# sxyu/volrend

Measured on AMD Instinct MI355X. Metric: Mrays/s at 800x800, NeRF-synthetic-like SH16 (synthetic C1), higher is better.
Workload: dtype f32; 1 GPU; C1: synthetic lego-like PlenOctree, depth 9, SH16, 2025715 nodes, 2.24 GB in HBM, 800x800, fx=fy=1111.111, 200-pose orbit, default RenderOptions; fp_mode=strict, launches=38, pcie_inclusive=False, launch_streams=1, parallelism=single GPU

## Files before the change

### include/volrend_hip.h

```cpp
#ifndef VOLREND_HIP_H_
#define VOLREND_HIP_H_

#include <stddef.h>
#include <stdint.h>

#ifdef __cplusplus
extern "C" {
#endif

#define VR_ABI_VERSION 3

enum {
    VR_OK = 0,
    VR_ERR_INVALID_ARGUMENT = 1,
    VR_ERR_HIP = 2,
    VR_ERR_NO_DEVICE = 3,
    VR_ERR_BAD_TREE = 4,
    VR_ERR_UNSUPPORTED = 5,
    VR_ERR_OUT_OF_MEMORY = 6
};

enum { VR_FORMAT_RGBA = 0, VR_FORMAT_SH = 1, VR_FORMAT_SG = 2, VR_FORMAT_ASG = 3 };

enum { VR_FP_STRICT = 0, VR_FP_FMA = 1 };
// ... 258 lines not shown
    int          bits;
    uint32_t*    order;
    uint32_t*    keys;
    float*       origins_out;
    float*       dirs_out;
    const float* payload;
    float*       payload_out;
    int          payload_dim;
} VrRayOrder;
int64_t vr_order_rays_workspace(int64_t n);
int vr_order_rays(vr_tree_t tree, int64_t n, const VrRays* rays, const VrRenderOptions* opt, int fp_mode,
                  const VrRayOrder* out, void* workspace, size_t workspace_bytes, void* stream);
int vr_reserve_rays(vr_tree_t tree, int64_t n, int n_slots);
int vr_reserve(vr_tree_t tree, int width, int height, int n_frames);
int vr_reserve_tiles(vr_tree_t tree, int width, int height, int n_frames, int tile_w, int tile_h,
                     int world, int n_slots);
int vr_tree_status(vr_tree_t tree, uint32_t* status, int reset);
int vr_tree_status_on(vr_tree_t tree, uint32_t* status, int reset, void* stream);
int vr_set_tuning(const char* key, int value);
int vr_tree_set_tuning(vr_tree_t tree, const char* key, int value);
int vr_sched_stats(vr_tree_t tree, uint64_t out[8], int reset);
int vr_tree_cull_stats(vr_tree_t tree, uint64_t out[2], int reset);
int vr_tree_head_stats(vr_tree_t tree, uint64_t out[3], int reset);
int vr_touch_enable(vr_tree_t tree, int enable);
int vr_touch_count(vr_tree_t tree, uint64_t out[4], int reset);
int vr_touch_read(vr_tree_t tree, int which, uint32_t* host_words, uint64_t n_words,
                  uint64_t* bitmap_words, uint64_t* granule_bytes);
int vr_assemble_tiles(void* frame_rgba, int64_t pitch, const void* gathered, int width,
                      int height, int tile_w, int tile_h, int world, void* stream);
int vr_assemble_tiles_batch(void* frames_rgba, int64_t frame_stride, int64_t pitch,
                            const void* gathered, int64_t rank_stride, int64_t in_frame_stride,
                            int n_frames, int width, int height, int tile_w, int tile_h, int world,
                            void* stream);
int vr_probe_coeffs(vr_tree_t tree, const VrRenderOptions* opt, float* out_dev, void* stream);

enum { VR_SPACE_WORLD = 0, VR_SPACE_TREE = 1 };

typedef struct VrQueryOut {
    float* sigma;
    int32_t* depth;
    float* local;
    float* coeffs;
    float* rgb;
} VrQueryOut;

int vr_query_points(vr_tree_t tree, int64_t n, const float* xyz_dev, const float* dirs_dev, int space,
// ... 13 lines not shown
```

### volrend_amd/_abi.py

```python
from __future__ import annotations

import ctypes as C
import os

HERE = os.path.dirname(os.path.abspath(__file__))
LIB_PATH = os.environ.get("VOLREND_HIP_LIB") or os.path.join(HERE, "libvolrend_hip.so")

VR_OK = 0
FORMAT_RGBA, FORMAT_SH, FORMAT_SG, FORMAT_ASG = 0, 1, 2, 3
FORMATS = {"RGBA": FORMAT_RGBA, "SH": FORMAT_SH, "SG": FORMAT_SG, "ASG": FORMAT_ASG}
FP_STRICT, FP_FMA = 0, 1
QUERY_LOOKUP, QUERY_DESCENT = 0, 1
LAYOUT_FRAME, LAYOUT_COMPACT = 0, 1
SPACE_WORLD, SPACE_TREE = 0, 1
SPACES = {"world": SPACE_WORLD, "tree": SPACE_TREE}
DEPTH_TREE, DEPTH_WORLD = 0, 1
DEPTH_UNITS = {"tree": DEPTH_TREE, "world": DEPTH_WORLD}
DATA_F16, DATA_F32 = 0, 1
STEP_SGD, STEP_ADAM = 0, 1
STEP_KINDS = {"sgd": STEP_SGD, "adam": STEP_ADAM}
MAX_BASIS = 25
ORDER_MAX_BITS, ORDER_MAX_PAYLOAD = 5, 8
REFINE_COPY, REFINE_ZERO = 0, 1
REFINE_FILLS = {"copy": REFINE_COPY, "zero": REFINE_ZERO}
# ... 173 lines not shown
    "vr_slot_points": (C.c_int, [C.POINTER(VrSlotPoints), C.c_void_p]),
    "vr_render_rays": (C.c_int, [C.c_void_p, C.c_int64, C.POINTER(VrRays), C.POINTER(VrRenderOptions), C.c_int,
                                 C.POINTER(VrRayOut), C.c_void_p]),
    "vr_accumulate_weights_rays": (C.c_int, [C.c_void_p, C.c_int64, C.POINTER(VrRays), C.POINTER(VrRenderOptions),
                                             C.c_int, C.POINTER(VrLeafWeights), C.c_void_p]),
    "vr_render_backward_rays": (C.c_int, [C.c_void_p, C.c_int64, C.POINTER(VrRays), C.POINTER(VrRenderOptions),
                                          C.c_int, C.c_void_p, C.c_void_p, C.c_void_p]),
    "vr_fit_rays": (C.c_int, [C.c_void_p, C.c_int64, C.POINTER(VrRays), C.POINTER(VrRenderOptions), C.c_int,
                              C.POINTER(VrFit), C.c_void_p]),
    "vr_order_rays_workspace": (C.c_int64, [C.c_int64]),
    "vr_order_rays": (C.c_int, [C.c_void_p, C.c_int64, C.POINTER(VrRays), C.POINTER(VrRenderOptions), C.c_int,
                                C.POINTER(VrRayOrder), C.c_void_p, C.c_size_t, C.c_void_p]),
    "vr_reserve_rays": (C.c_int, [C.c_void_p, C.c_int64, C.c_int]),
    "vr_reserve": (C.c_int, [C.c_void_p, C.c_int, C.c_int, C.c_int]),
    "vr_reserve_tiles": (C.c_int, [C.c_void_p, C.c_int, C.c_int, C.c_int, C.c_int, C.c_int, C.c_int,
                                   C.c_int]),
    "vr_tree_status": (C.c_int, [C.c_void_p, C.POINTER(C.c_uint32), C.c_int]),
    "vr_tree_status_on": (C.c_int, [C.c_void_p, C.POINTER(C.c_uint32), C.c_int, C.c_void_p]),
    "vr_set_tuning": (C.c_int, [C.c_char_p, C.c_int]),
    "vr_tree_set_tuning": (C.c_int, [C.c_void_p, C.c_char_p, C.c_int]),
    "vr_sched_stats": (C.c_int, [C.c_void_p, C.POINTER(C.c_uint64 * 8), C.c_int]),
    "vr_tree_cull_stats": (C.c_int, [C.c_void_p, C.POINTER(C.c_uint64 * 2), C.c_int]),
    "vr_tree_head_stats": (C.c_int, [C.c_void_p, C.POINTER(C.c_uint64 * 3), C.c_int]),
    "vr_touch_enable": (C.c_int, [C.c_void_p, C.c_int]),
    "vr_touch_count": (C.c_int, [C.c_void_p, C.POINTER(C.c_uint64 * 4), C.c_int]),
    "vr_touch_read": (C.c_int, [C.c_void_p, C.c_int, C.c_void_p, C.c_uint64, C.POINTER(C.c_uint64),
                                C.POINTER(C.c_uint64)]),
    "vr_assemble_tiles": (C.c_int, [C.c_void_p, C.c_int64, C.c_void_p, C.c_int, C.c_int, C.c_int,
                                    C.c_int, C.c_int, C.c_void_p]),
    "vr_assemble_tiles_batch": (C.c_int, [C.c_void_p, C.c_int64, C.c_int64, C.c_void_p, C.c_int64,
                                          C.c_int64, C.c_int, C.c_int, C.c_int, C.c_int, C.c_int,
                                          C.c_int, C.c_void_p]),
    "vr_probe_coeffs": (C.c_int, [C.c_void_p, C.POINTER(VrRenderOptions), C.c_void_p, C.c_void_p]),
    "vr_query_points": (C.c_int, [C.c_void_p, C.c_int64, C.c_void_p, C.c_void_p, C.c_int,
                                  C.POINTER(VrQueryOut), C.c_void_p]),
    "vr_query_grid": (C.c_int, [C.c_void_p, C.POINTER(C.c_float * 3), C.POINTER(C.c_float * 3),
                                C.POINTER(C.c_int32 * 3), C.POINTER(C.c_float * 3), C.c_int,
                                C.POINTER(VrQueryOut), C.c_void_p]),
    "vr_read_back": (C.c_int, [C.c_void_p, C.c_void_p, C.c_int64, C.c_int, C.c_int, C.c_void_p]),
    "vr_stream_sync": (C.c_int, [C.c_void_p]),
}

_lib = None


class VolrendError(RuntimeError):
# ... 27 lines not shown
```

### volrend_amd/_tree.py

```python
from __future__ import annotations

import ctypes as C
import os

import numpy as np

from . import _abi, _ops
from ._args import F16, I32, Buf, _stream_ptr, check


class _CurrentDevice:

    def info(self) -> dict:
        import torch
        return {"device": int(torch.cuda.current_device())}


def parse_data_format(s: str):
    idx = next((i for i, ch in enumerate(s) if not ch.isalpha()), -1)
    if idx < 0:
        return "RGBA", -1
    head = s[:idx]
    try:
        dim = int("".join(ch for ch in s[idx:] if ch.isdigit() or ch == "-") or "0")
# ... 211 lines not shown
        return self._loaded

    def clear_cpu_memory(self) -> None:
        self.data_ = None
        self.quant_ = None

    def sched_stats(self, reset: bool = True) -> dict:
        out = (C.c_uint64 * 8)()
        _abi.check(_abi.lib().vr_sched_stats(self._handle, C.byref(out), 1 if reset else 0))
        names = ("march_rounds", "march_lanes", "shade_rounds", "shade_lanes", "distinct_leaves",
                 "retire_rounds", "retired", "iterations")
        return dict(zip(names, [int(v) for v in out]))

    def cull_stats(self, reset: bool = True) -> dict:
        out = (C.c_uint64 * 2)()
        _abi.check(_abi.lib().vr_tree_cull_stats(self.handle, C.byref(out), 1 if reset else 0))
        return {"blocks": int(out[0]), "culled": int(out[1])}

    def head_stats(self, reset: bool = False) -> dict:
        out = (C.c_uint64 * 3)()
        _abi.check(_abi.lib().vr_tree_head_stats(self.handle, C.byref(out), 1 if reset else 0))
        return {"entered": int(out[0]), "retired": int(out[1]), "samples": int(out[2])}

    def touch_enable(self, enable: bool = True) -> None:
        _abi.check(_abi.lib().vr_touch_enable(self.handle, 1 if enable else 0))

    def touch_count(self, reset: bool = True) -> dict:
        out = (C.c_uint64 * 4)()
        _abi.check(_abi.lib().vr_touch_count(self.handle, C.byref(out), 1 if reset else 0))
        return dict(zip(("leaves", "nodes", "top", "bricks"), [int(v) for v in out]))

    def touch_read(self, which: int):
        words, gran = C.c_uint64(0), C.c_uint64(0)
        _abi.check(_abi.lib().vr_touch_read(self.handle, int(which), None, 0, C.byref(words), C.byref(gran)))
        out = np.zeros(int(words.value), dtype=np.uint32)
        if out.size:
            _abi.check(_abi.lib().vr_touch_read(self.handle, int(which), out.ctypes.data, out.size, None, None))
        return out, int(gran.value)

    def reserve(self, width: int, height: int, n_frames: int, shard: "TileShard | None" = None,
                n_slots: int = 2) -> None:
        if shard is None and n_slots == 2:
            _abi.check(_abi.lib().vr_reserve(self.handle, int(width), int(height), int(n_frames)))
        else:
            tw, th, world = (shard.tile_w, shard.tile_h, shard.world) if shard else (0, 0, 1)
            _abi.check(_abi.lib().vr_reserve_tiles(self.handle, int(width), int(height),
# ... 88 lines not shown
```

### volrend_amd/build.py

```python
from __future__ import annotations

import os
import shutil
import subprocess
import sys
import tempfile

HERE = os.path.dirname(os.path.abspath(__file__))
ROOT = os.path.dirname(HERE)
CSRC = os.path.join(HERE, "csrc")
LIB = os.path.join(HERE, "libvolrend_hip.so")
SOURCES = ["vr_render.hip", "vr_weights.hip", "vr_grad.hip", "vr_fit.hip", "vr_update.hip", "vr_tree_kernels.hip", "vr_query.hip", "vr_order.hip", "vr_refine.hip", "vr_collapse.hip", "vr_geometry.hip", "vr_api.cpp", "vr_upload.cpp", "vr_tree_walk.cpp",
           "vr_h2d.cpp", "vr_launch.cpp", "vr_launch_plan.cpp", "vr_slots.cpp", "vr_values.cpp", "vr_query.cpp", "vr_order.cpp", "vr_refine.cpp", "vr_collapse.cpp", "vr_geometry.cpp"]
HEADERS = ["vr_internal.h", "vr_device_math.h", "vr_host.h", "vr_dev_layout.h", "vr_dev_shade.h", "vr_dev_query.h",
           "vr_dev_rays.h", "vr_dev_march.h", "vr_dev_backward.h", "vr_query.h", "vr_order.h", "vr_refine.h", "vr_collapse.h", "vr_geometry.h", "vr_tree_walk.h", "vr_launch_plan.h", "vr_h2d.h", os.path.join(ROOT, "include", "volrend_hip.h"),
           os.path.join(ROOT, "include", "volrend", "internal", "hip_owners.hpp")]
EXPERIMENTS = os.path.join(ROOT, "tools", "experiments")
HOOK_FLAGS = ("-DVR_ABLATE", "-DVR_TIMELINE", "-DVR_ROLE_DEBUG", "-DVR_MIN_WAVES_PER_EU", "-DVR_SH16_ROWS",
              "-DVR_SHADE_SCHED_BARRIER", "-DVR_SH16_WAVES", "-DVR_SH25_WAVES", "-DVR_SH9_WAVES", "-DVR_PACKED_EXP",
              "-DVR_STEAL_MIN", "-DVR_EXP_SH25_STRIDE", "-DVR_TOUCH_LEAF_SHIFT")
HIPCC = os.environ.get("HIPCC", "/opt/rocm/bin/hipcc")
FLAGS = [
    "--offload-arch=gfx950", "-O3", "-std=c++17", "-fPIC", "-shared",
    "-ffp-contract=off",
    "-fhip-fp32-correctly-rounded-divide-sqrt",
    "-fno-gpu-flush-denormals-to-zero",
    "-fno-fast-math",
    "-x", "hip",
]


def needs_build() -> bool:
    if not os.path.exists(LIB):
        return True
    t = os.path.getmtime(LIB)
    deps = [os.path.join(CSRC, s) for s in SOURCES] + [
        h if os.path.isabs(h) else os.path.join(CSRC, h) for h in HEADERS]
    return any(os.path.getmtime(d) > t for d in deps)
# ... 48 lines not shown
```

### volrend_amd/csrc/vr_api.cpp

```cpp
#include <hip/hip_runtime.h>

#include <climits>
#include <cstdarg>
#include <cstdio>
#include <cstdlib>
#include <cstring>
#include <mutex>

#include "vr_host.h"
#include "vr_tree_walk.h"

namespace {

thread_local char g_err[512] = "";

enum KnobRange { kClamp, kClamp64, kFlag, kAutoFlag };
struct Knob { const char *key, *env; int Tuning::*field; KnobRange range; int lo, hi; bool fixed_at_upload; };
const Knob kKnobs[] = {
    {"march_max", "VR_MARCH_MAX", &Tuning::march_max, kClamp, 1, INT_MAX, false},
    {"refill_min", "VR_REFILL_MIN", &Tuning::refill_min, kClamp, 1, 64, false},
    {"drain_flush", "VR_DRAIN_FLUSH", &Tuning::drain_flush, kClamp, 0, 64, false},
    {"waves_per_cu", "VR_WAVES_PER_CU", &Tuning::waves_per_cu, kClamp, 0, 64, false},
    {"frame_group", "VR_FRAME_GROUP", &Tuning::frame_group, kClamp, 0, INT_MAX, false},
    {"super_block", "VR_SUPER_BLOCK", &Tuning::super_block, kClamp, 0, 64, false},
// ... 189 lines not shown
    HIP_TRY(hipMemcpy(lines, t->cull_stats.get(), sizeof(lines), hipMemcpyDeviceToHost));
    if (reset) HIP_TRY(hipMemset(t->cull_stats.get(), 0, sizeof(lines)));
    out[0] = out[1] = 0;
    for (int i = 0; i < vr::kCullStatLines; ++i) {
        out[0] += lines[i * vr::kCullStatStride];
        out[1] += lines[i * vr::kCullStatStride + 1];
    }
    return VR_OK;
}

int vr_tree_head_stats(vr_tree_t t, uint64_t out[3], int reset) {
    if (!t || !out) return fail(VR_ERR_INVALID_ARGUMENT, "NULL argument");
    DeviceGuard guard(t->device);
    uint64_t lines[vr::kCullStatLines * vr::kCullStatStride];
    HIP_TRY(hipMemcpy(lines, t->head_stats.get(), sizeof(lines), hipMemcpyDeviceToHost));
    if (reset) HIP_TRY(hipMemset(t->head_stats.get(), 0, sizeof(lines)));
    for (int k = 0; k < vr::kHeadStatWords; ++k) {
        out[k] = 0;
        for (int i = 0; i < vr::kCullStatLines; ++i) out[k] += lines[i * vr::kCullStatStride + k];
    }
    return VR_OK;
}

int vr_tree_status(vr_tree_t t, uint32_t* status, int reset) {
    if (!t || !status) return fail(VR_ERR_INVALID_ARGUMENT, "NULL argument");
    DeviceGuard guard(t->device);
    HIP_TRY(hipMemcpy(status, t->status.get(), sizeof(uint32_t), hipMemcpyDeviceToHost));
    if (reset) HIP_TRY(hipMemset(t->status.get(), 0, sizeof(uint32_t)));
    return VR_OK;
}

int vr_tree_status_on(vr_tree_t t, uint32_t* status, int reset, void* stream) {
    if (!t || !status) return fail(VR_ERR_INVALID_ARGUMENT, "NULL argument");
    DeviceGuard guard(t->device);
    hipStream_t hs = static_cast<hipStream_t>(stream);
    thread_local uint32_t* pinned = nullptr;
    if (!pinned) HIP_TRY(hipHostMalloc((void**)&pinned, sizeof(uint32_t), hipHostMallocPortable));
    HIP_TRY(hipMemcpyAsync(pinned, t->status.get(), sizeof(uint32_t), hipMemcpyDeviceToHost, hs));
    if (reset) HIP_TRY(hipMemsetAsync(t->status.get(), 0, sizeof(uint32_t), hs));
    HIP_TRY(hipStreamSynchronize(hs));
    *status = *pinned;
    return VR_OK;
}

int vr_touch_enable(vr_tree_t t, int enable) {
    if (!t) return fail(VR_ERR_INVALID_ARGUMENT, "tree is NULL");
// ... 103 lines not shown
```

### volrend_amd/csrc/vr_dev_march.h

```cpp
#pragma once
#include <type_traits>
#include "vr_device_math.h"
#include "vr_internal.h"
#include "vr_dev_layout.h"
#include "vr_dev_query.h"
#include "vr_dev_rays.h"

namespace vr {

namespace {

enum { kQueryN2 = 0, kQueryN2Blocked = 1, kQueryGeneric = 2 };
inline int query_kind(const KParams& p) {
    return !uses_lookup(p) ? kQueryGeneric : (p.brick_blocked ? kQueryN2Blocked : kQueryN2);
}
template <typename F>
void dispatch_query(int query, F&& f) {
    if (query == kQueryGeneric) f(std::integral_constant<int, kQueryGeneric>());
    else if (query == kQueryN2Blocked) f(std::integral_constant<int, kQueryN2Blocked>());
    else f(std::integral_constant<int, kQueryN2>());
}

struct WeightRecord {
    static constexpr int kWords = kWeightRayWords;
    static constexpr bool kShade = false;
};
struct GradRecord {
    static constexpr int kWords = kGradRayWords;
    static constexpr bool kShade = true;
};

template <int GW, typename Record>
__device__ __forceinline__ void store_march_record(const KParams& p, bool valid, int lane, int wave, const Ray& nr,
                                                   const float* vdir, uint32_t pixel) {
    const unsigned long long m_valid = __builtin_amdgcn_ballot_w64(valid);
    const uint32_t my_base = reserve_ray_slots<GW>(p, m_valid, lane, wave);
    if (!valid) return;
    uint32_t* rb = ray_slot(p.ray_buf_rw, Record::kWords, my_base + lane_rank(m_valid));
    store_march_words(rb, nr);
    if constexpr (Record::kShade) {
#pragma unroll
        for (int i = 0; i < 3; ++i) ray_word(rb, kGradRayVdir + i) = f2u(vdir[i]);
        ray_word(rb, kGradRayPixel) = pixel;
    }
}

template <int FMA, int GW, typename Record>
__global__ __launch_bounds__(kWave* GW) void march_raygen_kernel(const KParams p) {
    const int lane = threadIdx.x & (kWave - 1);
    const int wave = threadIdx.x >> 6;
    const uint32_t id = (uint32_t)(((int64_t)blockIdx.x * GW + wave) * kWave + lane);
    bool valid = false;
    Ray nr;
    nr.alive = false;
    float vdir[3] = {0.f, 0.f, 0.f};
    uint32_t pixel = 0;
    if (id < p.total_rays) {
        const PixelRef r = locate(p, id);
        if (r.in_image) {
            setup_ray<FMA>(p, r, nr, vdir);
            valid = nr.alive;
            pixel = ((uint32_t)r.frame * (uint32_t)p.height + (uint32_t)r.y) * (uint32_t)p.width + (uint32_t)r.x;
        }
    }
    store_march_record<GW, Record>(p, valid, lane, wave, nr, vdir, pixel);
}

template <int FMA, int GW, typename Record>
__global__ __launch_bounds__(kWave* GW) void march_raygen_rays_kernel(const KParams p, const RayList rl) {
    const int lane = threadIdx.x & (kWave - 1);
    const int wave = threadIdx.x >> 6;
    uint32_t id;
    Ray nr;
    float vdir[3] = {0.f, 0.f, 0.f};
    const bool valid = list_ray<FMA, GW>(p, rl, lane, wave, id, nr, vdir) && nr.alive;
    store_march_record<GW, Record>(p, valid, lane, wave, nr, vdir, id);
}

template <typename Launch>
void launch_raygen_waves(const KParams& p, int gen_waves, Launch&& launch) {
    const int gw = gen_waves >= 16 ? 16 : 4;
    const dim3 grid((unsigned)((p.n_wave_blocks * p.n_frames + gw - 1) / gw)), block(kWave * gw);
    if (gw == 16) launch(std::integral_constant<int, 16>(), grid, block);
    else launch(std::integral_constant<int, 4>(), grid, block);
}
template <int FMA, typename Record>
void launch_march_raygen(const KParams& p, int gen_waves, hipStream_t s, const RayList* rays) {
    launch_raygen_waves(p, gen_waves, [&](auto gw, dim3 grid, dim3 block) {
        constexpr int GW = decltype(gw)::value;
        if (rays) hipLaunchKernelGGL((march_raygen_rays_kernel<FMA, GW, Record>), grid, block, 0, s, p, *rays);
        else hipLaunchKernelGGL((march_raygen_kernel<FMA, GW, Record>), grid, block, 0, s, p);
    });
}

struct MarchFeed {
    bool exhausted;
    uint32_t chunk_next, chunk_end;
    uint32_t progress_round;
};
// ... 132 lines not shown
```

### volrend_amd/csrc/vr_dev_rays.h

```cpp
#pragma once
#include "vr_device_math.h"
#include "vr_dev_layout.h"
#include "vr_dev_shade.h"

namespace vr {

namespace {

struct RayCounters {
    uint32_t samples = 0, child_reads = 0, hits = 0, early = 0, entered = 0;
};

typedef __attribute__((address_space(1))) uint32_t vr_gword_t;
typedef float vr_f4_t __attribute__((ext_vector_type(4)));
typedef __attribute__((address_space(1))) vr_f4_t vr_gfloat4_t;

__device__ __forceinline__ bool wave_any(bool v) { return __builtin_amdgcn_ballot_w64(v) != 0ull; }
__device__ __forceinline__ uint32_t lane_id_now() {
    uint32_t l;
    asm volatile("v_mbcnt_lo_u32_b32 %0, -1, 0\n\tv_mbcnt_hi_u32_b32 %0, -1, %0" : "=v"(l));
    return l;
}
__device__ __forceinline__ uint32_t lane_rank(unsigned long long mask) {
    return __builtin_amdgcn_mbcnt_hi((uint32_t)(mask >> 32), __builtin_amdgcn_mbcnt_lo((uint32_t)mask, 0u));
}

// ... 265 lines not shown
            const uint32_t x = (mine + a) & (nq - 1u);
            uint32_t* const q = p.queue_head + x * kQueueStride;
            uint32_t* const head = q + kQueueHead;
            const uint32_t len = q[kQueueCount];
            const uint32_t seen = __hip_atomic_load(head, __ATOMIC_RELAXED, __HIP_MEMORY_SCOPE_AGENT);
            if (seen >= len) continue;
            if (a != 0u && gridDim.x >= nq &&
                len - seen < ((len >> 3) < kStealMin ? (len >> 3) : kStealMin))
                continue;
            uint32_t size = (len - seen) / (2u * waves_per_q);
            size = size < 64u ? 64u : (size > (uint32_t)p.chunk_max ? (uint32_t)p.chunk_max : size);
            size &= ~63u;
            const uint32_t base = atomicAdd(head, size);
            if (base < len) {
                const uint32_t qlo = queue_first_block(n16, x, sh) << 6;
                lo = qlo + base;
                hi = qlo + (base + size < len ? base + size : len);
                break;
            }
        }
    }
}

template <int GW>
__device__ __forceinline__ uint32_t reserve_ray_slots(const KParams& p, unsigned long long m_valid, int lane,
                                                      int wave) {
    __shared__ uint32_t wave_count[GW];
    __shared__ uint32_t wave_base[GW];
    const uint32_t nq = (uint32_t)p.n_queues;
    uint32_t sh, n16;
    queue_split(p, sh, n16);
    const uint32_t g16 = (uint32_t)(((int64_t)blockIdx.x * GW) >> 4);
    uint32_t qx = (uint32_t)(((uint64_t)g16 << sh) / n16);
    while (qx + 1u < nq && (queue_first_block(n16, qx + 1u, sh) >> 4) <= g16) ++qx;
    while (qx > 0u && (queue_first_block(n16, qx, sh) >> 4) > g16) --qx;
    uint32_t* const q_count = p.queue_head + qx * kQueueStride + kQueueCount;
    const uint32_t q_base = queue_first_block(n16, qx, sh) << 6;
    if constexpr (GW == 1) {
        const uint32_t n = (uint32_t)__builtin_popcountll(m_valid);
        uint32_t b = 0;
        if (lane == 0 && n) b = atomicAdd(q_count, n);
        return q_base + (uint32_t)__builtin_amdgcn_readfirstlane((int)b);
    } else {
        if (lane == 0) wave_count[wave] = (uint32_t)__builtin_popcountll(m_valid);
        __syncthreads();
        if (threadIdx.x == 0) {
            uint32_t sum = 0;
#pragma unroll
            for (int w = 0; w < GW; ++w) {
                wave_base[w] = sum;
                sum += wave_count[w];
            }
            const uint32_t base = q_base + (sum ? atomicAdd(q_count, sum) : 0u);
#pragma unroll
            for (int w = 0; w < GW; ++w) wave_base[w] += base;
        }
        __syncthreads();
        return wave_base[wave];
    }
}

__device__ __forceinline__ void store_march_words(uint32_t* rb, const Ray& nr) {
#pragma unroll
    for (int i = 0; i < 3; ++i) {
        ray_word(rb, kRayCen + i) = f2u(nr.cen[i]);
        ray_word(rb, kRayDir + i) = f2u(nr.dir[i]);
        ray_word(rb, kRayInvDir + i) = f2u(nr.invdir[i]);
    }
    ray_word(rb, kRayT) = f2u(nr.t);
    ray_word(rb, kRayTmax) = f2u(nr.tmax);
    ray_word(rb, kRayDeltaScale) = f2u(nr.delta_scale);
}

template <int FMA, int GW>
__device__ __forceinline__ bool list_ray(const KParams& p, const RayList& rl, int lane, int wave, uint32_t& id,
                                         Ray& ray, float* vdir) {
    typedef __attribute__((address_space(1))) const float vr_gcfloat_t;
    __shared__ float tr[GW][2][3 * kWave];
    const int64_t first = ((int64_t)blockIdx.x * GW + wave) * kWave;
    const int64_t left = rl.n - first;
    const int count = left <= 0 ? 0 : (left < kWave ? (int)left : kWave);
    vr_gcfloat_t* const so = (vr_gcfloat_t*)rl.origins + first * 3;
    vr_gcfloat_t* const sd = (vr_gcfloat_t*)rl.dirs + first * 3;
#pragma unroll
    for (int c = 0; c < 3; ++c) {
        const int f = c * kWave + lane;
        if (f < count * 3) {
            tr[wave][0][f] = so[f];
            tr[wave][1][f] = sd[f];
        }
    }
    __syncthreads();
    id = (uint32_t)first + (uint32_t)lane;
    reset_ray(ray);
    if (lane >= count) return false;
    if (p.N <= 0) return true;
    float cen[3], dir[3];
#pragma unroll
    for (int c = 0; c < 3; ++c) {
        cen[c] = tr[wave][0][lane * 3 + c];
        dir[c] = tr[wave][1][lane * 3 + c];
    }
// ... 9 lines not shown
```

### volrend_amd/csrc/vr_fit.hip

```cpp
#include "vr_dev_backward.h"

namespace vr {

namespace {

__device__ __forceinline__ void loss_head(const FitParams& fp, uint32_t i, const float* out, float* g) {
    vr_gcfloat_t* const tg = (vr_gcfloat_t*)fp.target + (size_t)i * 3u;
    const float na = 1.f - out[3];
    float r[3];
#pragma unroll
    for (int ch = 0; ch < 3; ++ch) {
        const float pred = out[ch] + fp.bg * na;
        r[ch] = pred - tg[ch];
    }
    if (fp.sq_err) ((vr_gfloat_t*)fp.sq_err)[i] = (r[0] * r[0] + r[1] * r[1]) + r[2] * r[2];
    if (fp.accum) ((vr_gfloat4_t*)fp.accum)[i] = (vr_f4_t){out[0], out[1], out[2], out[3]};
#pragma unroll
    for (int ch = 0; ch < 3; ++ch) g[ch] = fp.grad_scale * r[ch];
    g[3] = -(fp.bg * ((g[0] + g[1]) + g[2]));
}

template <int FMA, int GW>
__global__ __launch_bounds__(kWave* GW) void fit_raygen_kernel(const KParams p, const RayList rl, const FitParams fp) {
    const int lane = threadIdx.x & (kWave - 1);
    const int wave = threadIdx.x >> 6;
    uint32_t id;
    Ray nr;
    float vdir[3] = {0.f, 0.f, 0.f};
    const bool has = list_ray<FMA, GW>(p, rl, lane, wave, id, nr, vdir);
    const bool valid = has && nr.alive;
    if (has && !valid) {
        const float out[4] = {0.f, 0.f, 0.f, 0.f};
        float g[4];
        loss_head(fp, id, out, g);
    }
    store_march_record<GW, GradRecord>(p, valid, lane, wave, nr, vdir, id);
}

struct FitArgs : FitParams {
    static constexpr bool kFit = true, kMark = true;
    explicit FitArgs(const FitParams& f) : FitParams(f) {}
};

template <int FMA>
hipError_t launch_fp(const KParams& p, const FitParams& fp, int n_cus, int waves_override, int gen_waves, hipStream_t s,
                     const RayList& rays) {
    launch_raygen_waves(p, gen_waves, [&](auto gw, dim3 grid, dim3 block) {
        hipLaunchKernelGGL((fit_raygen_kernel<FMA, decltype(gw)::value>), grid, block, 0, s, p, rays, fp);
    });
    return launch_backward_march<FMA>(p, FitArgs(fp), n_cus, waves_override, s);
}

}

hipError_t launch_fit(const KParams& p, const FitParams& fp, int fp_mode, int n_cus, int waves_override, int gen_waves,
                      hipStream_t stream, const RayList* rays) {
    if (p.n_wave_blocks <= 0 || p.n_frames <= 0 || !rays) return hipSuccess;
    return fp_mode == VR_FP_FMA ? launch_fp<1>(p, fp, n_cus, waves_override, gen_waves, stream, *rays)
                                : launch_fp<0>(p, fp, n_cus, waves_override, gen_waves, stream, *rays);
// ... 4 lines not shown
```

### volrend_amd/csrc/vr_host.h

```cpp
#pragma once
#include <hip/hip_runtime.h>

#include <mutex>
#include <vector>

#include "vr_internal.h"
#include "vr_launch_plan.h"

#pragma GCC visibility push(hidden)

#include "volrend/internal/hip_owners.hpp"
using volrend::internal::DeviceBuffer;
using volrend::internal::DeviceEvent;
using volrend::internal::DeviceGuard;

int fail(int code, const char* fmt, ...);
inline int hip_code(hipError_t e) { return e == hipErrorOutOfMemory ? VR_ERR_OUT_OF_MEMORY : VR_ERR_HIP; }

#define HIP_TRY(expr)                                                                                 \
    do {                                                                                              \
        hipError_t e_ = (expr);                                                                       \
        if (e_ != hipSuccess)                                                                         \
            return fail(hip_code(e_), "%s failed: %s (%s:%d)", #expr, hipGetErrorString(e_), __FILE__, \
                        __LINE__);                                                                    \
// ... 23 lines not shown
    uint64_t device_bytes = 0;
};

struct VrTreeOpaque : TreeShape {
    int device = 0;
    DeviceBuffer arrays[4];
    DeviceBuffer extra, status, sched_stats;
    DeviceBuffer occ;
    DeviceBuffer cull_stats;
    DeviceBuffer head_stats;
    DeviceBuffer touch[4];
    DeviceBuffer touch_out;
    DeviceBuffer probe_buf;
    DeviceBuffer slot_frames;
    DeviceBuffer slot_heads;
    DeviceBuffer slot_aovs;
    std::vector<int32_t> file_node;
    DeviceBuffer file_node_dev;
    std::vector<int32_t> brick_root;
    DeviceBuffer brick_root_dev;
    DeviceBuffer node_of_file_dev;
    LaunchSlot slots[kLaunchSlots];
    unsigned launch_seq = 0;
    std::mutex launch_mutex;
    Tuning tn;
    int n_cus = 256;
};

void fill_tree_params(vr::KParams& k, const VrTreeOpaque* t);

int tile_geometry(int width, int height, int tile_w, int tile_h, int rank, int world, vr::KParams& k);
int launch_geometry(int width, int height, int tile_w, int tile_h, int rank, int world, int n_frames,
                    vr::KParams& k);
int list_geometry(const char* what, int64_t n, vr::KParams& k);

inline size_t ray_buffer_bytes(uint32_t total_rays, int words_per_ray) {
    return vr::ray_slots(total_rays) * (size_t)words_per_ray * sizeof(uint32_t);
}
inline size_t list_pixel_bytes(uint32_t total_rays) { return (size_t)total_rays * 4; }
inline uint32_t block_mask_words(const vr::KParams& k) {
    const uint64_t blocks = (uint64_t)k.tiles_x * (uint64_t)(k.tile_w / 8) * (uint64_t)k.tiles_y * (uint64_t)(k.tile_h / 8);
    return (uint32_t)(((blocks + 127) / 128) * 4);
}
inline size_t block_mask_bytes(const vr::KParams& k, int n_frames) {
    return (size_t)block_mask_words(k) * sizeof(uint32_t) * (size_t)n_frames;
}
// ... 19 lines not shown
```

### volrend_amd/csrc/vr_order.hip

```cpp
#include <cstring>

#include <rocprim/device/device_radix_sort.hpp>

#include "vr_dev_rays.h"
#include "vr_order.h"

namespace vr {

namespace {

__device__ __forceinline__ uint32_t order_quant(float v, float scale) {
    const float s = v * scale;
    return s > 0.f ? (uint32_t)vmin(s, scale - 1.f) : 0u;
}

__device__ __forceinline__ uint32_t order_morton(const uint32_t* q, int bits) {
    uint32_t key = 0;
    for (int b = 0; b < bits; ++b) {
#pragma unroll
        for (int c = 0; c < 6; ++c) key |= ((q[c] >> b) & 1u) << (6 * b + c);
    }
    return key;
}

template <int FMA, int GW>
__global__ __launch_bounds__(kWave* GW) void order_key_kernel(const KParams p, const RayList rl, const OrderArgs a) {
    using P = Policy<FMA>;
    const int lane = threadIdx.x & (kWave - 1), wave = threadIdx.x >> 6;
    uint32_t id;
    Ray ray;
    float vdir[3];
    if (!list_ray<FMA, GW>(p, rl, lane, wave, id, ray, vdir)) return;
    uint32_t key = kOrderMissKey;
    if (ray.entered) {
        const float scale = (float)(1 << a.bits);
        uint32_t q[6];
#pragma unroll
        for (int c = 0; c < 3; ++c) {
            q[c] = order_quant(P::madd(ray.t, ray.dir[c], ray.cen[c]), scale);
            q[3 + c] = order_quant(P::madd(ray.tmax, ray.dir[c], ray.cen[c]), scale);
        }
        key = order_morton(q, a.bits);
    }
    a.key[0][id] = key;
    a.idx[0][id] = id;
}

__device__ __forceinline__ void gather_rows(const float* src, float* dst, int dim, uint32_t from, int64_t first,
                                            int count, float* rows) {
    const int lane = threadIdx.x;
    if (lane < count) {
        const float* const s = src + (size_t)from * (size_t)dim;
        for (int c = 0; c < dim; ++c) rows[lane * dim + c] = s[c];
    }
    __syncthreads();
// ... 53 lines not shown
```

### volrend_amd/csrc/vr_render.hip

```cpp
#include "vr_device_math.h"
#include "vr_internal.h"
#include "vr_dev_layout.h"
#include "vr_dev_shade.h"
#include "vr_dev_query.h"
#include "vr_dev_rays.h"
#include "vr_dev_march.h"

namespace vr {

namespace {

constexpr int kSh16Waves = 5;
constexpr int kSh25Waves = 4;
constexpr int kSh9Waves = 7;
constexpr int kSh16Rows = 64;

constexpr int kRing = 128;

template <int BASIS>
struct Stage {
    static constexpr bool kEnabled = BASIS > 1;
    static constexpr int kVec = kEnabled ? RecTraits<BASIS>::kDwords / 4 : 1;
    static constexpr int kRow = kVec * 16;
    static constexpr int kPerInstr = kWave / kVec;
// ... 457 lines not shown
    }
    if (COUNT && p.sched_stats && lane == 0) {
        atomicAdd(&p.sched_stats[kStatMarchRounds], (unsigned long long)st_march_r);
        atomicAdd(&p.sched_stats[kStatMarchLanes], (unsigned long long)st_march_l);
        atomicAdd(&p.sched_stats[kStatShadeRounds], (unsigned long long)st_shade_r);
        atomicAdd(&p.sched_stats[kStatShadeLanes], (unsigned long long)st_shade_l);
        atomicAdd(&p.sched_stats[kStatDistinctLeaves], (unsigned long long)st_distinct);
        atomicAdd(&p.sched_stats[kStatRetireRounds], (unsigned long long)st_fin_r);
        atomicAdd(&p.sched_stats[kStatRetiredRays], (unsigned long long)st_fin_l);
        atomicAdd(&p.sched_stats[kStatIterations], (unsigned long long)st_iter);
    }
}



template <int FMA, bool FULL, int GW, bool HEAD, typename... PLANES>
__global__ __launch_bounds__(kWave* GW)
void raygen_kernel(const KParams p, const PLANES... planes, const CullParams cull, const HeadParams head) {
    static_assert(!(HEAD && FULL), "the FULL flavours count every sample in the march kernel");
    constexpr bool AOV = sizeof...(PLANES) != 0;
    const AovParams aov = aov_arg(planes...);
    const int lane = threadIdx.x & (kWave - 1);
    const int wave = threadIdx.x >> 6;
    const uint32_t id =
        (uint32_t)(((int64_t)blockIdx.x * GW + wave) * kWave + lane);
    bool valid = false;
    bool culled = false;
    Ray nr;
    uint8_t* px = nullptr;
    uint32_t xy = 0;
    int frame = 0;
    float vdir[3] = {0.f, 0.f, 1.f};
    auto keep_or_finish = [&]() {
        if (nr.alive) {
            valid = true;
        } else {
            RayCounters z;
            finish_ray<FMA, FULL>(p, nr, z, px, xy, frame);
            if constexpr (AOV) store_aov(aov, frame, xy, 0.f, 1.f);
        }
    };
    bool has = false;
    if constexpr (HEAD) nr.alive = false;
    if (id < p.total_rays) {
        const PixelRef r = locate(p, id);
        if constexpr (!FULL) {
            if (cull.mask) {
                const uint32_t b = (uint32_t)(r.y >> 3) * cull.nbx + (uint32_t)(r.x >> 3);
// ... 9 lines not shown
            else setup_ray<FMA>(p, r, nr, vdir);
            if constexpr (HEAD) has = true;
            else keep_or_finish();
        }
    }
    uint32_t head_n[kHeadStatWords] = {0u, 0u, 0u};
    if constexpr (HEAD) {
        head_n[0] = (uint32_t)__builtin_popcountll(__builtin_amdgcn_ballot_w64(nr.alive));
        if (head_n[0] != 0u)
            head_n[2] = p.brick_blocked ? head_march<FMA, kQueryN2Blocked>(p, head, nr)
                                        : head_march<FMA, kQueryN2>(p, head, nr);
        head_n[1] = head_n[0] - (uint32_t)__builtin_popcountll(__builtin_amdgcn_ballot_w64(nr.alive));
        if (has) keep_or_finish();
    }
    const unsigned long long m_valid = __builtin_amdgcn_ballot_w64(valid);
    __shared__ uint32_t wave_culled[GW];
    __shared__ uint32_t wave_head[HEAD ? GW : 1][kHeadStatWords];
    if constexpr (!FULL && GW > 1) {
        if (cull.mask && lane == 0) wave_culled[wave] = culled ? 1u : 0u;
        if constexpr (HEAD) {
            if (lane < kHeadStatWords) wave_head[wave][lane] = lane == 0 ? head_n[0] : lane == 1 ? head_n[1] : head_n[2];
        }
    }
    const uint32_t my_base = reserve_ray_slots<GW>(p, m_valid, lane, wave);
    if constexpr (!FULL) {
        if (cull.mask && threadIdx.x < 2u) {
            const int64_t left = (int64_t)(p.total_rays >> 6) - (int64_t)blockIdx.x * GW;
            uint32_t n = (uint32_t)(left < 0 ? 0 : (left < GW ? left : GW));
            if (threadIdx.x == 1u) {
                if constexpr (GW > 1) {
                    n = 0;
#pragma unroll
                    for (int w = 0; w < GW; ++w) n += wave_culled[w];
                } else {
                    n = culled ? 1u : 0u;
                }
            }
            if (n)
                atomicAdd(cull.stats + (blockIdx.x & (uint32_t)(kCullStatLines - 1)) * kCullStatStride + threadIdx.x,
                          (unsigned long long)n);
        }
    }
    if constexpr (HEAD) {
        if (threadIdx.x < (uint32_t)kHeadStatWords) {
            uint32_t n = 0;
            if constexpr (GW > 1) {
#pragma unroll
                for (int w = 0; w < GW; ++w) n += wave_head[w][threadIdx.x];
            } else {
                n = threadIdx.x == 0u ? head_n[0] : threadIdx.x == 1u ? head_n[1] : head_n[2];
// ... 21 lines not shown
    ray_word(rb, kRayFrame) = (uint32_t)frame;
    if (p.ray_vdir) {
#pragma unroll
        for (int i = 0; i < 3; ++i) ray_word(rb, kRayTail + i) = f2u(vdir[i]);
    } else if (p.basis_words > 0) {
        float b[VR_MAX_BASIS];
#pragma unroll
        for (int i = 0; i < VR_MAX_BASIS; ++i) b[i] = 0.f;
        precalc_basis<FMA, FULL>(p, vdir, b);
#pragma unroll
        for (int i = 0; i < VR_MAX_BASIS; ++i)
            if (i < p.basis_words)
                ray_word(rb, kRayTail + i) = f2u((i < p.basis_min || i > p.basis_max) ? 0.f : b[i]);
    }
}

template <int FMA, bool FULL, int GW>
__global__ __launch_bounds__(kWave* GW) void raygen_rays_kernel(const KParams p, const RayList rl) {
    const int lane = threadIdx.x & (kWave - 1);
    const int wave = threadIdx.x >> 6;
    uint32_t id;
    Ray nr;
    float vdir[3] = {0.f, 0.f, 1.f};
    const bool has = list_ray<FMA, GW>(p, rl, lane, wave, id, nr, vdir);
    bool valid = false;
    uint8_t* px = nullptr;
    uint32_t xy = 0;
    if (has) {
        xy = (id & (uint32_t)(kRayListWidth - 1)) | ((id >> kRayListShift) << 16);
        px = p.frames[0].rgba + (int64_t)id * 4;
        if (nr.alive) {
            valid = true;
        } else {
            RayCounters z;
            finish_ray<FMA, false>(p, nr, z, px, xy, 0);
        }
    }
    const unsigned long long m_valid = __builtin_amdgcn_ballot_w64(valid);
    const uint32_t my_base = reserve_ray_slots<GW>(p, m_valid, lane, wave);
    if (!valid) return;
    store_colour_ray<FMA, FULL>(p, my_base + lane_rank(m_valid), nr, xy, px, 0, vdir);
}

__global__ void prepare_launch_kernel(FrameTable tbl, FrameDesc* frames, uint32_t* queue_head, uint32_t* mask,
                                      uint32_t words_per_frame) {
    const int i = threadIdx.x;
    if (i < tbl.n) frames[tbl.first + i] = tbl.f[i];
    if (tbl.first == 0 && i < kMaxQueues) {
        queue_head[i * kQueueStride + kQueueHead] = 0u;
        queue_head[i * kQueueStride + kQueueCount] = 0u;
    }
    if (mask) {
        uint4* const q = reinterpret_cast<uint4*>(mask + (size_t)tbl.first * words_per_frame);
        const uint32_t n = (uint32_t)tbl.n * (words_per_frame >> 2);
        for (uint32_t j = threadIdx.x; j < n; j += blockDim.x) q[j] = make_uint4(0u, 0u, 0u, 0u);
    }
}

__global__ __launch_bounds__(256) void block_mask_kernel(const KParams p, const MaskParams m) {
    __shared__ uint32_t bits[kMaskMaxWords];
    __shared__ uint32_t whole;
    const uint32_t wpf = m.words_per_frame;
// ... 265 lines not shown
```

### volrend_amd/csrc/vr_slots.cpp

```cpp
#include <hip/hip_runtime.h>

#include <mutex>

#include "vr_host.h"

namespace {

hipError_t replace_ray_buffer(LaunchSlot& ls, size_t bytes) {
    if (ls.rays) {
        if (ls.used) (void)hipEventSynchronize(ls.done.get());
        (void)ls.rays.reset();
        (void)hipGetLastError();
    }
    return ls.rays.alloc(bytes);
}

int reserve_slots(VrTreeOpaque* t, int n_slots, size_t need) {
    DeviceGuard device_guard(t->device);
    std::lock_guard<std::mutex> guard(t->launch_mutex);
    for (int i = 0; i < n_slots; ++i) {
        LaunchSlot& ls = t->slots[i];
        if (ls.growing || ls.rays.bytes() >= need) continue;
        const hipError_t e = replace_ray_buffer(ls, need);
        if (e != hipSuccess) return fail(hip_code(e), "ray buffer of %zu bytes: %s", need, hipGetErrorString(e));
// ... 12 lines not shown
                 size_t need, unsigned& slot) {
    slot = kLaunchSlots;
    for (int want_fit = 1; want_fit >= 0 && slot == kLaunchSlots; --want_fit) {
        for (int pass = 0; pass < 2 && slot == kLaunchSlots; ++pass)
            for (unsigned i = 0; i < kLaunchSlots; ++i) {
                const LaunchSlot& c = t->slots[i];
                if (c.growing || (want_fit && c.rays.bytes() < need)) continue;
                const bool ok = pass == 0 ? (c.used && c.last_stream == hs)
                                          : (!c.used || hipEventQuery(c.done.get()) == hipSuccess);
                if (ok) {
                    slot = i;
                    break;
                }
            }
    }
    (void)hipGetLastError();
    if (slot == kLaunchSlots) {
        for (unsigned a = 0; a < kLaunchSlots && slot == kLaunchSlots; ++a)
            if (!t->slots[(t->launch_seq + a) % kLaunchSlots].growing) slot = (t->launch_seq + a) % kLaunchSlots;
        if (slot == kLaunchSlots)
            return fail(VR_ERR_HIP, "all %u launch slots are being resized by other threads", kLaunchSlots);
    }
    t->launch_seq++;
    LaunchSlot& ls = t->slots[slot];
    k.frames = t->slot_frames.get<vr::FrameDesc>() + (size_t)slot * vr::kMaxBatch;
    k.queue_head = t->slot_heads.get<uint32_t>() + vr::kSlotWords * slot + vr::kSlotHeaderWords;
    k.probe_coeffs = t->probe_buf.get<float>() + (size_t)slot * (size_t)t->desc.data_dim;
    if (ls.rays.bytes() < need) {
        ls.growing = true;
        guard.unlock();
        const hipError_t ge = replace_ray_buffer(ls, need);
        guard.lock();
        ls.growing = false;
        if (ge != hipSuccess)
            return fail(hip_code(ge), "ray buffer of %zu bytes: %s", need, hipGetErrorString(ge));
    }
    k.ray_buf_rw = ls.rays.get<uint32_t>();
    k.ray_buf = k.ray_buf_rw;
    return VR_OK;
}

int SlotTurn::begin(LaunchSlot& ls, hipStream_t hs) {
    if (ls.used) HIP_TRY(hipStreamWaitEvent(hs, ls.done.get(), 0));
    slot_ = &ls;
    stream_ = hs;
    return VR_OK;
// ... 42 lines not shown
```

Before: 3041 Mrays/s.

## Interleave raygen workgroups across the eight ray queues

Raygen blocks are remapped so consecutive block indices round-robin across the 8 per-queue regions instead of filling one queue at a time. The likely aim is to spread atomic reservation traffic on the queue counters and to fill all queues early, so downstream marching can start on every queue. It adds an index-mapping function with a tail loop for uneven queue sizes, and a host query for per-queue counts. Ray-to-block locality changes, which may affect cache behaviour during raygen.

```diff
diff --git a/include/volrend_hip.h b/include/volrend_hip.h
--- a/include/volrend_hip.h
+++ b/include/volrend_hip.h
@@ -304,6 +304,7 @@
 int vr_sched_stats(vr_tree_t tree, uint64_t out[8], int reset);
 int vr_tree_cull_stats(vr_tree_t tree, uint64_t out[2], int reset);
 int vr_tree_head_stats(vr_tree_t tree, uint64_t out[3], int reset);
+int vr_tree_queue_counts(vr_tree_t tree, uint32_t out[8]);
 int vr_touch_enable(vr_tree_t tree, int enable);
 int vr_touch_count(vr_tree_t tree, uint64_t out[4], int reset);
 int vr_touch_read(vr_tree_t tree, int which, uint32_t* host_words, uint64_t n_words,
diff --git a/volrend_amd/_abi.py b/volrend_amd/_abi.py
--- a/volrend_amd/_abi.py
+++ b/volrend_amd/_abi.py
@@ -219,6 +219,7 @@
     "vr_sched_stats": (C.c_int, [C.c_void_p, C.POINTER(C.c_uint64 * 8), C.c_int]),
     "vr_tree_cull_stats": (C.c_int, [C.c_void_p, C.POINTER(C.c_uint64 * 2), C.c_int]),
     "vr_tree_head_stats": (C.c_int, [C.c_void_p, C.POINTER(C.c_uint64 * 3), C.c_int]),
+    "vr_tree_queue_counts": (C.c_int, [C.c_void_p, C.POINTER(C.c_uint32 * 8)]),
     "vr_touch_enable": (C.c_int, [C.c_void_p, C.c_int]),
     "vr_touch_count": (C.c_int, [C.c_void_p, C.POINTER(C.c_uint64 * 4), C.c_int]),
     "vr_touch_read": (C.c_int, [C.c_void_p, C.c_int, C.c_void_p, C.c_uint64, C.POINTER(C.c_uint64),
diff --git a/volrend_amd/_tree.py b/volrend_amd/_tree.py
--- a/volrend_amd/_tree.py
+++ b/volrend_amd/_tree.py
@@ -257,6 +257,11 @@
         _abi.check(_abi.lib().vr_tree_head_stats(self.handle, C.byref(out), 1 if reset else 0))
         return {"entered": int(out[0]), "retired": int(out[1]), "samples": int(out[2])}
 
+    def queue_counts(self) -> list:
+        out = (C.c_uint32 * 8)()
+        _abi.check(_abi.lib().vr_tree_queue_counts(self.handle, C.byref(out)))
+        return [int(v) for v in out]
+
     def touch_enable(self, enable: bool = True) -> None:
         _abi.check(_abi.lib().vr_touch_enable(self.handle, 1 if enable else 0))
 
diff --git a/volrend_amd/build.py b/volrend_amd/build.py
--- a/volrend_amd/build.py
+++ b/volrend_amd/build.py
@@ -13,7 +13,7 @@
 SOURCES = ["vr_render.hip", "vr_weights.hip", "vr_grad.hip", "vr_fit.hip", "vr_update.hip", "vr_tree_kernels.hip", "vr_query.hip", "vr_order.hip", "vr_refine.hip", "vr_collapse.hip", "vr_geometry.hip", "vr_api.cpp", "vr_upload.cpp", "vr_tree_walk.cpp",
            "vr_h2d.cpp", "vr_launch.cpp", "vr_launch_plan.cpp", "vr_slots.cpp", "vr_values.cpp", "vr_query.cpp", "vr_order.cpp", "vr_refine.cpp", "vr_collapse.cpp", "vr_geometry.cpp"]
 HEADERS = ["vr_internal.h", "vr_device_math.h", "vr_host.h", "vr_dev_layout.h", "vr_dev_shade.h", "vr_dev_query.h",
-           "vr_dev_rays.h", "vr_dev_march.h", "vr_dev_backward.h", "vr_query.h", "vr_order.h", "vr_refine.h", "vr_collapse.h", "vr_geometry.h", "vr_tree_walk.h", "vr_launch_plan.h", "vr_h2d.h", os.path.join(ROOT, "include", "volrend_hip.h"),
+           "vr_dev_rays.h", "vr_queue_map.h", "vr_dev_march.h", "vr_dev_backward.h", "vr_query.h", "vr_order.h", "vr_refine.h", "vr_collapse.h", "vr_geometry.h", "vr_tree_walk.h", "vr_launch_plan.h", "vr_h2d.h", os.path.join(ROOT, "include", "volrend_hip.h"),
            os.path.join(ROOT, "include", "volrend", "internal", "hip_owners.hpp")]
 EXPERIMENTS = os.path.join(ROOT, "tools", "experiments")
 HOOK_FLAGS = ("-DVR_ABLATE", "-DVR_TIMELINE", "-DVR_ROLE_DEBUG", "-DVR_MIN_WAVES_PER_EU", "-DVR_SH16_ROWS",
diff --git a/volrend_amd/csrc/vr_api.cpp b/volrend_amd/csrc/vr_api.cpp
--- a/volrend_amd/csrc/vr_api.cpp
+++ b/volrend_amd/csrc/vr_api.cpp
@@ -235,6 +235,21 @@
     return VR_OK;
 }
 
+int vr_tree_queue_counts(vr_tree_t t, uint32_t out[vr::kMaxQueues]) {
+    if (!t || !out) return fail(VR_ERR_INVALID_ARGUMENT, "NULL argument");
+    DeviceGuard guard(t->device);
+    unsigned slot;
+    {
+        std::lock_guard<std::mutex> g(t->launch_mutex);
+        slot = t->last_slot;
+    }
+    uint32_t words[vr::kMaxQueues * vr::kQueueStride];
+    HIP_TRY(hipMemcpy(words, t->slot_heads.get<uint32_t>() + vr::kSlotWords * slot + vr::kSlotHeaderWords, sizeof(words),
+                      hipMemcpyDeviceToHost));
+    for (int x = 0; x < vr::kMaxQueues; ++x) out[x] = words[x * vr::kQueueStride + vr::kQueueCount];
+    return VR_OK;
+}
+
 int vr_tree_status(vr_tree_t t, uint32_t* status, int reset) {
     if (!t || !status) return fail(VR_ERR_INVALID_ARGUMENT, "NULL argument");
     DeviceGuard guard(t->device);
diff --git a/volrend_amd/csrc/vr_dev_march.h b/volrend_amd/csrc/vr_dev_march.h
--- a/volrend_amd/csrc/vr_dev_march.h
+++ b/volrend_amd/csrc/vr_dev_march.h
@@ -31,10 +31,10 @@
 };
 
 template <int GW, typename Record>
-__device__ __forceinline__ void store_march_record(const KParams& p, bool valid, int lane, int wave, const Ray& nr,
-                                                   const float* vdir, uint32_t pixel) {
+__device__ __forceinline__ void store_march_record(const KParams& p, const BlockGroup& bg, bool valid, int lane, int wave,
+                                                   const Ray& nr, const float* vdir, uint32_t pixel) {
     const unsigned long long m_valid = __builtin_amdgcn_ballot_w64(valid);
-    const uint32_t my_base = reserve_ray_slots<GW>(p, m_valid, lane, wave);
+    const uint32_t my_base = reserve_ray_slots<GW>(p, m_valid, lane, wave, bg);
     if (!valid) return;
     uint32_t* rb = ray_slot(p.ray_buf_rw, Record::kWords, my_base + lane_rank(m_valid));
     store_march_words(rb, nr);
@@ -49,7 +49,8 @@
 __global__ __launch_bounds__(kWave* GW) void march_raygen_kernel(const KParams p) {
     const int lane = threadIdx.x & (kWave - 1);
     const int wave = threadIdx.x >> 6;
-    const uint32_t id = (uint32_t)(((int64_t)blockIdx.x * GW + wave) * kWave + lane);
+    const BlockGroup bg = raygen_block_group<GW>(p);
+    const uint32_t id = (uint32_t)(((int64_t)bg.group * GW + wave) * kWave + lane);
     bool valid = false;
     Ray nr;
     nr.alive = false;
@@ -63,7 +64,7 @@
             pixel = ((uint32_t)r.frame * (uint32_t)p.height + (uint32_t)r.y) * (uint32_t)p.width + (uint32_t)r.x;
         }
     }
-    store_march_record<GW, Record>(p, valid, lane, wave, nr, vdir, pixel);
+    store_march_record<GW, Record>(p, bg, valid, lane, wave, nr, vdir, pixel);
 }
 
 template <int FMA, int GW, typename Record>
@@ -73,8 +74,9 @@
     uint32_t id;
     Ray nr;
     float vdir[3] = {0.f, 0.f, 0.f};
-    const bool valid = list_ray<FMA, GW>(p, rl, lane, wave, id, nr, vdir) && nr.alive;
-    store_march_record<GW, Record>(p, valid, lane, wave, nr, vdir, id);
+    const BlockGroup bg = raygen_block_group<GW>(p);
+    const bool valid = list_ray<FMA, GW>(p, rl, bg.group, lane, wave, id, nr, vdir) && nr.alive;
+    store_march_record<GW, Record>(p, bg, valid, lane, wave, nr, vdir, id);
 }
 
 template <typename Launch>
diff --git a/volrend_amd/csrc/vr_dev_rays.h b/volrend_amd/csrc/vr_dev_rays.h
--- a/volrend_amd/csrc/vr_dev_rays.h
+++ b/volrend_amd/csrc/vr_dev_rays.h
@@ -2,6 +2,7 @@
 #include "vr_device_math.h"
 #include "vr_dev_layout.h"
 #include "vr_dev_shade.h"
+#include "vr_queue_map.h"
 
 namespace vr {
 
@@ -313,20 +314,24 @@
     }
 }
 
+static_assert(kSpreadQueues == (uint32_t)kMaxQueues, "vr_queue_map.h restates the queue count of vr_internal.h");
+template <int GW>
+__device__ __forceinline__ BlockGroup raygen_block_group(const KParams& p) {
+    static_assert(GW == 1 || GW == 2 || GW == 4 || GW == 8 || GW == 16, "a workgroup never straddles a queue boundary");
+    constexpr uint32_t gw_log2 = GW == 1 ? 0u : GW == 2 ? 1u : GW == 4 ? 2u : GW == 8 ? 3u : 4u;
+    const uint32_t sh = (uint32_t)p.n_queues == (uint32_t)kMaxQueues ? (uint32_t)kMaxQueuesShift : 0u;
+    return spread_block_group(blockIdx.x, p.total_rays >> 6, sh, gw_log2);
+}
+
 template <int GW>
 __device__ __forceinline__ uint32_t reserve_ray_slots(const KParams& p, unsigned long long m_valid, int lane,
-                                                      int wave) {
+                                                      int wave, const BlockGroup& bg) {
     __shared__ uint32_t wave_count[GW];
     __shared__ uint32_t wave_base[GW];
-    const uint32_t nq = (uint32_t)p.n_queues;
     uint32_t sh, n16;
     queue_split(p, sh, n16);
-    const uint32_t g16 = (uint32_t)(((int64_t)blockIdx.x * GW) >> 4);
-    uint32_t qx = (uint32_t)(((uint64_t)g16 << sh) / n16);
-    while (qx + 1u < nq && (queue_first_block(n16, qx + 1u, sh) >> 4) <= g16) ++qx;
-    while (qx > 0u && (queue_first_block(n16, qx, sh) >> 4) > g16) --qx;
-    uint32_t* const q_count = p.queue_head + qx * kQueueStride + kQueueCount;
-    const uint32_t q_base = queue_first_block(n16, qx, sh) << 6;
+    uint32_t* const q_count = p.queue_head + bg.queue * kQueueStride + kQueueCount;
+    const uint32_t q_base = queue_first_block(n16, bg.queue, sh) << 6;
     if constexpr (GW == 1) {
         const uint32_t n = (uint32_t)__builtin_popcountll(m_valid);
         uint32_t b = 0;
@@ -364,11 +369,11 @@
 }
 
 template <int FMA, int GW>
-__device__ __forceinline__ bool list_ray(const KParams& p, const RayList& rl, int lane, int wave, uint32_t& id,
-                                         Ray& ray, float* vdir) {
+__device__ __forceinline__ bool list_ray(const KParams& p, const RayList& rl, uint32_t group, int lane, int wave,
+                                         uint32_t& id, Ray& ray, float* vdir) {
     typedef __attribute__((address_space(1))) const float vr_gcfloat_t;
     __shared__ float tr[GW][2][3 * kWave];
-    const int64_t first = ((int64_t)blockIdx.x * GW + wave) * kWave;
+    const int64_t first = ((int64_t)group * GW + wave) * kWave;
     const int64_t left = rl.n - first;
     const int count = left <= 0 ? 0 : (left < kWave ? (int)left : kWave);
     vr_gcfloat_t* const so = (vr_gcfloat_t*)rl.origins + first * 3;
diff --git a/volrend_amd/csrc/vr_fit.hip b/volrend_amd/csrc/vr_fit.hip
--- a/volrend_amd/csrc/vr_fit.hip
+++ b/volrend_amd/csrc/vr_fit.hip
@@ -27,14 +27,15 @@
     uint32_t id;
     Ray nr;
     float vdir[3] = {0.f, 0.f, 0.f};
-    const bool has = list_ray<FMA, GW>(p, rl, lane, wave, id, nr, vdir);
+    const BlockGroup bg = raygen_block_group<GW>(p);
+    const bool has = list_ray<FMA, GW>(p, rl, bg.group, lane, wave, id, nr, vdir);
     const bool valid = has && nr.alive;
     if (has && !valid) {
         const float out[4] = {0.f, 0.f, 0.f, 0.f};
         float g[4];
         loss_head(fp, id, out, g);
     }
-    store_march_record<GW, GradRecord>(p, valid, lane, wave, nr, vdir, id);
+    store_march_record<GW, GradRecord>(p, bg, valid, lane, wave, nr, vdir, id);
 }
 
 struct FitArgs : FitParams {
diff --git a/volrend_amd/csrc/vr_host.h b/volrend_amd/csrc/vr_host.h
--- a/volrend_amd/csrc/vr_host.h
+++ b/volrend_amd/csrc/vr_host.h
@@ -69,6 +69,7 @@
     DeviceBuffer node_of_file_dev;
     LaunchSlot slots[kLaunchSlots];
     unsigned launch_seq = 0;
+    unsigned last_slot = 0;
     std::mutex launch_mutex;
     Tuning tn;
     int n_cus = 256;
diff --git a/volrend_amd/csrc/vr_order.hip b/volrend_amd/csrc/vr_order.hip
--- a/volrend_amd/csrc/vr_order.hip
+++ b/volrend_amd/csrc/vr_order.hip
@@ -30,7 +30,7 @@
     uint32_t id;
     Ray ray;
     float vdir[3];
-    if (!list_ray<FMA, GW>(p, rl, lane, wave, id, ray, vdir)) return;
+    if (!list_ray<FMA, GW>(p, rl, blockIdx.x, lane, wave, id, ray, vdir)) return;
     uint32_t key = kOrderMissKey;
     if (ray.entered) {
         const float scale = (float)(1 << a.bits);
diff --git a/volrend_amd/csrc/vr_queue_map.h b/volrend_amd/csrc/vr_queue_map.h
--- /dev/null
+++ b/volrend_amd/csrc/vr_queue_map.h
@@ -0,0 +1,55 @@
+#pragma once
+#include <cstdint>
+
+#if defined(__HIPCC__)
+#define VR_QMAP_FN __host__ __device__ inline
+#define VR_QMAP_NOUNROLL _Pragma("nounroll")
+#else
+#define VR_QMAP_FN inline
+#define VR_QMAP_NOUNROLL
+#endif
+
+namespace vr {
+
+constexpr uint32_t kSpreadQueues = 8;
+
+VR_QMAP_FN uint32_t queue_first_group16(uint32_t n16, uint32_t x, uint32_t sh) {
+    return (uint32_t)(((uint64_t)n16 * x) >> sh);
+}
+
+struct BlockGroup {
+    uint32_t group;
+    uint32_t queue;
+};
+
+VR_QMAP_FN BlockGroup spread_block_group(uint32_t b, uint32_t n_blocks, uint32_t sh, uint32_t gw_log2) {
+    BlockGroup r = {b, 0u};
+    const uint32_t n_groups = (n_blocks + (1u << gw_log2) - 1u) >> gw_log2;
+    if (sh == 0u || b >= n_groups) return r;
+    const uint32_t n16 = (n_blocks + 15u) >> 4, per16 = 4u - gw_log2;
+    uint32_t least = (n16 >> sh) << per16;
+    if ((n16 & (kSpreadQueues - 1u)) == 0u) least -= (n16 << per16) - n_groups;
+    if (b < least * kSpreadQueues) {
+        const uint32_t round = b >> 3;
+        r.queue = (b + round) & (kSpreadQueues - 1u);
+        r.group = (queue_first_group16(n16, r.queue, sh) << per16) + round;
+        return r;
+    }
+    uint32_t k = b - least * kSpreadQueues;
+    VR_QMAP_NOUNROLL
+    for (uint32_t x = 0; x < kSpreadQueues; ++x) {
+        const uint32_t lo = queue_first_group16(n16, x, sh) << per16;
+        uint32_t hi = queue_first_group16(n16, x + 1u, sh) << per16;
+        hi = hi < n_groups ? hi : n_groups;
+        const uint32_t rest = hi - lo - least;
+        if (k < rest) {
+            r.group = lo + least + k;
+            r.queue = x;
+            return r;
+        }
+        k -= rest;
+    }
+    return r;
+}
+
+}
diff --git a/volrend_amd/csrc/vr_render.hip b/volrend_amd/csrc/vr_render.hip
--- a/volrend_amd/csrc/vr_render.hip
+++ b/volrend_amd/csrc/vr_render.hip
@@ -503,8 +503,8 @@
     const AovParams aov = aov_arg(planes...);
     const int lane = threadIdx.x & (kWave - 1);
     const int wave = threadIdx.x >> 6;
-    const uint32_t id =
-        (uint32_t)(((int64_t)blockIdx.x * GW + wave) * kWave + lane);
+    const BlockGroup bg = raygen_block_group<GW>(p);
+    const uint32_t id = (uint32_t)(((int64_t)bg.group * GW + wave) * kWave + lane);
     bool valid = false;
     bool culled = false;
     Ray nr;
@@ -560,10 +560,10 @@
             if (lane < kHeadStatWords) wave_head[wave][lane] = lane == 0 ? head_n[0] : lane == 1 ? head_n[1] : head_n[2];
         }
     }
-    const uint32_t my_base = reserve_ray_slots<GW>(p, m_valid, lane, wave);
+    const uint32_t my_base = reserve_ray_slots<GW>(p, m_valid, lane, wave, bg);
     if constexpr (!FULL) {
         if (cull.mask && threadIdx.x < 2u) {
-            const int64_t left = (int64_t)(p.total_rays >> 6) - (int64_t)blockIdx.x * GW;
+            const int64_t left = (int64_t)(p.total_rays >> 6) - (int64_t)bg.group * GW;
             uint32_t n = (uint32_t)(left < 0 ? 0 : (left < GW ? left : GW));
             if (threadIdx.x == 1u) {
                 if constexpr (GW > 1) {
@@ -631,7 +631,8 @@
     uint32_t id;
     Ray nr;
     float vdir[3] = {0.f, 0.f, 1.f};
-    const bool has = list_ray<FMA, GW>(p, rl, lane, wave, id, nr, vdir);
+    const BlockGroup bg = raygen_block_group<GW>(p);
+    const bool has = list_ray<FMA, GW>(p, rl, bg.group, lane, wave, id, nr, vdir);
     bool valid = false;
     uint8_t* px = nullptr;
     uint32_t xy = 0;
@@ -646,7 +647,7 @@
         }
     }
     const unsigned long long m_valid = __builtin_amdgcn_ballot_w64(valid);
-    const uint32_t my_base = reserve_ray_slots<GW>(p, m_valid, lane, wave);
+    const uint32_t my_base = reserve_ray_slots<GW>(p, m_valid, lane, wave, bg);
     if (!valid) return;
     store_colour_ray<FMA, FULL>(p, my_base + lane_rank(m_valid), nr, xy, px, 0, vdir);
 }
diff --git a/volrend_amd/csrc/vr_slots.cpp b/volrend_amd/csrc/vr_slots.cpp
--- a/volrend_amd/csrc/vr_slots.cpp
+++ b/volrend_amd/csrc/vr_slots.cpp
@@ -58,6 +58,7 @@
             return fail(VR_ERR_HIP, "all %u launch slots are being resized by other threads", kLaunchSlots);
     }
     t->launch_seq++;
+    t->last_slot = slot;
     LaunchSlot& ls = t->slots[slot];
     k.frames = t->slot_frames.get<vr::FrameDesc>() + (size_t)slot * vr::kMaxBatch;
     k.queue_head = t->slot_heads.get<uint32_t>() + vr::kSlotWords * slot + vr::kSlotHeaderWords;
```

After: 3002 Mrays/s. -1.3%, worse.
